# Sudaraka88/LDWeaver

Measured on AMD Instinct MI355X. Metric: MI SNP-pairs/sec, higher is better.
Workload: dtype i8

## Files before the change

### include/ldweaver_amd_debug.h

```cpp
#ifndef LDWEAVER_AMD_DEBUG_H
#define LDWEAVER_AMD_DEBUG_H

#include "ldweaver_amd.h"

#ifdef __cplusplus
extern "C" {
#endif

#define LDW_ENGINE_MFMA 0
#define LDW_ENGINE_HIST 1
#define LDW_ENGINE_HIST_STATES 2

int ldw_build_info(void);
int ldw_ctx_last_timing(ldw_ctx *ctx, double ms_out[4]);
int ldw_ctx_counters(ldw_ctx *ctx, int64_t out[4]);
int ldw_ctx_counters2(ldw_ctx *ctx, int64_t out[8]);
int ldw_gemm_stats(ldw_ctx *ctx, double out[6], int reset);
int ldw_apx_info(ldw_ctx *ctx, double out[6]);

int ldw_hamming_stats(ldw_ctx *ctx, double out[8]);
int ldw_joint_tables(ldw_ctx *ctx, const int32_t *pair_a, const int32_t *pair_b, int64_t npairs,
                     int64_t *counts_out, int64_t *fixed_out, int *frac_bits_out);

int ldw_set_engine(ldw_ctx *ctx, int engine);
int ldw_set_overlap(ldw_ctx *ctx, int on);
int ldw_set_fused(ldw_ctx *ctx, int on);
int ldw_set_mixed(ldw_ctx *ctx, int on);
int ldw_set_path(ldw_ctx *ctx, int mode);
int ldw_set_select(ldw_ctx *ctx, int mode);
int ldw_set_screen(ldw_ctx *ctx, int mode);
int ldw_set_prune(ldw_ctx *ctx, int on);
int ldw_set_pair_cap(uint32_t cap);
int ldw_reset_speculation(ldw_ctx *ctx);

int ldw_path_report(ldw_ctx *ctx, int64_t out[8], char *gate, int capacity);
int ldw_pair_form_report(ldw_ctx *ctx, int64_t out[5]);
int ldw_prune_report(ldw_ctx *ctx, int64_t out[4]);
int ldw_span_report(ldw_ctx *ctx, int64_t out[4]);
int ldw_overflow_report(ldw_ctx *ctx, int64_t out[4]);
int ldw_slot_report(ldw_ctx *ctx, int64_t out[6]);
int ldw_resource_report(int64_t out[5]);

int ldw_snp_bounds(ldw_ctx *ctx, double *out, int64_t capacity);
int ldw_debug_violations(ldw_ctx *ctx, double *out);
int ldw_debug_tab11(ldw_ctx *ctx, double W, double lo, double delta, double eta, double sprime, int32_t *out, double *cbin_out);
int ldw_debug_apx_params(ldw_ctx *ctx, double out[20], int64_t *vfixed_out, int64_t *vapx_out, int64_t capacity);
int ldw_debug_rows(ldw_ctx *ctx, int32_t *row0_out, uint32_t *slot_meta_out, int64_t capacity);
int ldw_debug_apx_gemm(ldw_ctx *ctx, const int32_t *rows_t, int nrt, const int32_t *rows_f, int nrf, int32_t *out);
int ldw_debug_apx_gemm_list(ldw_ctx *ctx, const int32_t *rows_t, int nrt, const int32_t *rows_f, int nrf, int grid_wgs, int32_t *out);
int ldw_debug_screen_bound(ldw_ctx *ctx, int kind, int na, int nb, int64_t n, const int64_t *g, const int64_t *pa, const int64_t *pb, const float *pX, const float *pY,
                           const double *rr, const uint32_t *masks, const double params[20], float *out, double *out64);

int ldw_debug_plot_panels(ldw_ctx *ctx, const double *x, const double *y, const double *srp, const uint8_t *layer, const uint8_t *panel, int64_t n,
                          int on_device, const ldw_plot_opts *opts, int n_panels, int32_t W, int32_t H, uint8_t *rgb_out, double *stats_out,
                          int64_t *scratch_bytes_out, double *ms_out);
int ldw_debug_plot_xy_panel(ldw_ctx *ctx, const double *x, const double *y, const uint8_t *cls, int64_t n, int on_device, const double *line_x,
                            const double *line_y, int64_t n_line, const ldw_plot_xy_opts *opts, int32_t W, int32_t H, uint8_t *rgb_out, double *stats_out,
                            double *ms_out);
int ldw_debug_plot_colours(int kind, const double *t, int64_t n, uint8_t *rgb_out);
int ldw_debug_plot_capsules(ldw_ctx *ctx, const ldw_capsule *caps, int64_t n_caps, int32_t W, int32_t H, uint8_t *rgb_out, double *ms_out);
int ldw_debug_plot_marks(ldw_ctx *ctx, const ldw_capsule *caps, int64_t n_caps, const ldw_rect *rects, int64_t n_rects, int32_t W, int32_t H, uint8_t *rgb_out,
                         double *ms_out);
int ldw_debug_plot_tree(ldw_ctx *ctx, int32_t W, int32_t H, const int32_t *panel, const ldw_bar *bars, int64_t n_bars, uint32_t bar_rgb, const uint8_t *levels,
                        int64_t n_tips, const uint32_t *palette, const int32_t *band_rect, int32_t n_bands, uint8_t *rgb_out, double *ms_out);
int ldw_links_grep_stats(ldw_ctx *ctx, double *out8);
int ldw_tsv_stats(ldw_ctx *ctx, double *out10);
int ldw_tsv_set_variant(ldw_ctx *ctx, int variant);

#ifdef __cplusplus
}
#endif
#endif
```

### ldweaver_amd/_lib.py

```python
from __future__ import annotations

import ctypes as C
import os

import numpy as np

_HERE = os.path.dirname(os.path.abspath(__file__))
LIB_PATH = os.environ.get("LDW_AMD_LIB") or os.path.join(_HERE, "libldweaver_amd.so")

LDW_OK = 0
LDW_ERR_ARG, LDW_ERR_HIP, LDW_ERR_STATE, LDW_ERR_NOGPU, LDW_ERR_SIZE = 1, 2, 3, 4, 5
QUIRK_REFERENCE, QUIRK_INTENDED = 0, 1
MI_SR_ROWS_STAY = 1
ENGINE_MFMA, ENGINE_HIST, ENGINE_HIST_STATES = 0, 1, 2
COL_INT32, COL_INT64, COL_DOUBLE, COL_STR = 0, 1, 2, 3


class LdwError(RuntimeError):
    def __init__(self, code: int, msg: str):
        super().__init__(f"libldweaver_amd error {code}: {msg}")
        self.code = code


PLOT_SR_CLUST, PLOT_SR_COMBI, PLOT_LR, PLOT_LDMAP = 0, 1, 2, 3
# ... 112 lines not shown
    "ldw_png_write": (C.c_int, [C.c_char_p, _p, C.c_int32, C.c_int32, C.c_int, C.POINTER(_i64)]),
    "ldw_plot_scatter": (C.c_int, [_p, _p, _p, _p, _p, _p, _i64, C.c_int, _p, C.c_int, _p, C.c_char_p, _p, C.POINTER(_i64)]),
    "ldw_plot_links": (C.c_int, [_p, C.c_int, C.c_int, _p, C.c_char_p, _p, C.POINTER(_i64)]),
    "ldw_plot_heatmap": (C.c_int, [_p, _p, C.c_int32, C.c_int, C.c_char_p, C.c_char_p, _p]),
    "ldw_plot_ldmap": (C.c_int, [_p, C.c_int32, C.c_int32, C.c_int32, C.c_char_p, C.c_char_p, _p, _p, _p, _p, _i64]),
    "ldw_plot_xy_layout_get": (C.c_int, [C.c_int, C.c_int, C.c_double, C.c_double, C.c_double, C.c_double, _p]),
    "ldw_plot_xy": (C.c_int, [_p, _p, _p, _p, _i64, C.c_int, _p, _p, _i64, _p, C.c_char_p, C.c_char_p, C.c_char_p, C.c_char_p, _p, C.POINTER(_i64)]),
    "ldw_plot_network": (C.c_int, [_p, _p, _i64, C.c_int32, C.c_int32, _p, _p, C.c_int32, C.c_char_p, _p, _p, C.c_int32, C.c_int32, C.c_char_p, _p, _p]),
    "ldw_plot_tanglegram": (C.c_int, [_p, _p, _i64, _p, _i64, C.c_int32, C.c_int32, _p, _p, C.c_int32, C.c_char_p, C.c_int32, C.c_char_p, _p, _p]),
    "ldw_plot_tree": (C.c_int, [_p, C.c_int32, C.c_int32, _p, _p, _i64, C.c_uint32, _p, _i64, _p, _p, C.c_int32, _p, C.c_char_p, _p, _p, _p, _p, _p, C.c_int32,
                                C.c_char_p, _p, _p]),
    "ldw_nj_tree": (C.c_int, [_p, _p, _i64, _p, _p]),
    "ldw_nj_bootstrap": (C.c_int, [_p, _p, _i64, _i64, _p, _p, _p, _p, _p]),
    "ldw_tree_parsimony": (C.c_int, [_p, _p, _p, _i64, C.c_int32, _p, _p]),
    "ldw_tree_states": (C.c_int, [_p, _p, _p, _i64, C.c_int32, _p, _i64, _p]),
    "ldw_tree_cochanges": (C.c_int, [_p, _p, _p, _i64, C.c_int32, _p, _p, _i64, _p, _p, _p]),
    "ldw_seq_clusters": (C.c_int, [_p, _p, C.c_int32, _p, _p]),
    "ldw_links_stratified": (C.c_int, [_p, _p, _p, _i64, _p, C.c_int32, _p, _p, _p, _p, _p, _p, C.POINTER(C.c_int)]),
    "ldw_links_permuted": (C.c_int, [_p, _p, _p, _i64, _p, C.c_int32, C.c_int32, C.c_uint64, _p, _p, _p, _p, _p, _p, C.POINTER(_i64), C.POINTER(C.c_int)]),
    "ldw_tsv_probe": (C.c_int, [C.c_char_p, C.c_int, C.POINTER(C.c_int32), C.POINTER(C.c_int32)]),
    "ldw_tsv_read": (C.c_int, [_p, C.c_char_p, C.c_int, C.c_int32, _i64, C.POINTER(_i64), C.POINTER(_i64), C.POINTER(C.c_uint32)]),
    "ldw_tsv_columns": (C.c_int, [_p, C.POINTER(_p), C.POINTER(_i64), C.POINTER(C.c_int32), C.POINTER(_i64)]),
    "ldw_tsv_fetch": (C.c_int, [_p, C.c_int32, _p, _i64, C.c_int]),
    "ldw_set_positions": (C.c_int, [_p, _p, _i64, C.c_double]),
    "ldw_links_load": (C.c_int, [_p, C.c_int, C.c_int32, C.c_int32, C.c_int32, C.c_int32, C.c_double, C.c_int32, C.POINTER(_i64)]),
    "ldw_links_grep": (C.c_int, [_p, C.c_char_p, _p, _p, C.c_int32, C.c_int32, _i64, C.POINTER(_i64), C.POINTER(_i64), C.POINTER(_i64)]),
    "ldw_links_grep_fetch": (C.c_int, [_p, _i64, _i64, _p, _p, _p, _p, _p]),
    "ldw_compare_to_row": (C.c_int, [_p, _i64, _i64, _p, _i64, _p]),
    "ldw_vec_pos_match": (C.c_int, [_p, _i64, _p, _i64, _p]),
    "ldw_compare_triplet": (C.c_int, [_p, _p, _i64, C.c_double, C.POINTER(C.c_int)]),
    "ldw_fast_intersect": (C.c_int, [_p, _i64, _p, _i64, _p, C.POINTER(_i64)]),
}
_SIGS_DEBUG = {
    "ldw_build_info": (C.c_int, []),
    "ldw_ctx_last_timing": (C.c_int, [_p, _p]),
    "ldw_ctx_counters": (C.c_int, [_p, _p]),
    "ldw_ctx_counters2": (C.c_int, [_p, _p]),
    "ldw_gemm_stats": (C.c_int, [_p, _p, C.c_int]),
    "ldw_apx_info": (C.c_int, [_p, _p]),
    "ldw_hamming_stats": (C.c_int, [_p, _p]),
    "ldw_joint_tables": (C.c_int, [_p, _p, _p, _i64, _p, _p, _p]),
    "ldw_set_engine": (C.c_int, [_p, C.c_int]),
    "ldw_set_overlap": (C.c_int, [_p, C.c_int]),
    "ldw_set_fused": (C.c_int, [_p, C.c_int]),
    "ldw_set_mixed": (C.c_int, [_p, C.c_int]),
    "ldw_set_path": (C.c_int, [_p, C.c_int]),
    "ldw_set_select": (C.c_int, [_p, C.c_int]),
    "ldw_set_screen": (C.c_int, [_p, C.c_int]),
    "ldw_set_prune": (C.c_int, [_p, C.c_int]),
    "ldw_set_pair_cap": (C.c_int, [C.c_uint32]),
    "ldw_reset_speculation": (C.c_int, [_p]),
    "ldw_path_report": (C.c_int, [_p, _p, C.c_char_p, C.c_int]),
    "ldw_pair_form_report": (C.c_int, [_p, _p]),
    "ldw_prune_report": (C.c_int, [_p, _p]),
    "ldw_span_report": (C.c_int, [_p, _p]),
    "ldw_overflow_report": (C.c_int, [_p, _p]),
    "ldw_slot_report": (C.c_int, [_p, _p]),
    "ldw_resource_report": (C.c_int, [_p]),
    "ldw_snp_bounds": (C.c_int, [_p, _p, C.c_int64]),
    "ldw_debug_violations": (C.c_int, [_p, _p]),
    "ldw_debug_tab11": (C.c_int, [_p, C.c_double, C.c_double, C.c_double, C.c_double, C.c_double, _p, _p]),
    "ldw_debug_apx_params": (C.c_int, [_p, _p, _p, _p, _i64]),
    "ldw_debug_rows": (C.c_int, [_p, _p, _p, _i64]),
    "ldw_debug_apx_gemm": (C.c_int, [_p, _p, C.c_int, _p, C.c_int, _p]),
    "ldw_debug_apx_gemm_list": (C.c_int, [_p, _p, C.c_int, _p, C.c_int, C.c_int, _p]),
    "ldw_debug_screen_bound": (C.c_int, [_p, C.c_int, C.c_int, C.c_int, _i64, _p, _p, _p, _p, _p, _p, _p, _p, _p, _p]),
    "ldw_debug_plot_panels": (C.c_int, [_p, _p, _p, _p, _p, _p, _i64, C.c_int, _p, C.c_int, C.c_int32, C.c_int32, _p, _p, C.POINTER(_i64), _p]),
    "ldw_debug_plot_xy_panel": (C.c_int, [_p, _p, _p, _p, _i64, C.c_int, _p, _p, _i64, _p, C.c_int32, C.c_int32, _p, _p, _p]),
    "ldw_debug_plot_colours": (C.c_int, [C.c_int, _p, _i64, _p]),
    "ldw_debug_plot_capsules": (C.c_int, [_p, _p, _i64, C.c_int32, C.c_int32, _p, _p]),
    "ldw_debug_plot_marks": (C.c_int, [_p, _p, _i64, _p, _i64, C.c_int32, C.c_int32, _p, _p]),
    "ldw_debug_plot_tree": (C.c_int, [_p, C.c_int32, C.c_int32, _p, _p, _i64, C.c_uint32, _p, _i64, _p, _p, C.c_int32, _p, _p]),
    "ldw_links_grep_stats": (C.c_int, [_p, _p]),
    "ldw_tsv_stats": (C.c_int, [_p, _p]),
    "ldw_tsv_set_variant": (C.c_int, [_p, C.c_int]),
}
_SIGS = {**_SIGS_API, **_SIGS_DEBUG}
_SIGS_BY_HEADER = {"ldweaver_amd.h": _SIGS_API, "ldweaver_amd_debug.h": _SIGS_DEBUG}


def declared_symbols(header: str | None = None):
    return sorted(_SIGS if header is None else _SIGS_BY_HEADER[header])


def lib():
    global _lib
    if _lib is None:
        if not os.path.exists(LIB_PATH):
            raise FileNotFoundError(
                f"{LIB_PATH} not found: build it with `make -C ldweaver_amd/csrc` or "
                "`python -c 'import __graft_entry__ as g; g.build()'` — there is no CPU fallback")
        try:
            import torch
        except ImportError:
            pass
        l = C.CDLL(LIB_PATH)
        for name, (res, args) in _SIGS.items():
            fn = getattr(l, name)
            fn.restype = res
            fn.argtypes = args
        _lib = l
    return _lib


def has_experiments() -> bool:
    return bool(lib().ldw_build_info() & 1)
# ... 23 lines not shown
```

### ldweaver_amd/csrc/ldw_api.hip

```cpp
#include <algorithm>
#include <atomic>
#include <chrono>
#include <cmath>
#include <cstdio>
#include <cstdlib>
#include <cstring>

#include <thread>
#include "ldw_internal.h"
#include "ldw_dev.h"
#include "ldw_fasta.h"
#include "ldw_links_read.h"
#include "ldw_slots.h"

namespace ldw {
int check_gpu(ldw_ctx *ctx) {
    LDW_REQUIRE(ctx != nullptr, LDW_ERR_ARG, "null context");
    LDW_HIP(hipSetDevice(ctx->device));
    return LDW_OK;
}
}

using namespace ldw;

// ... 316 lines not shown
        LDW_HIP(c->stream.ensure(hipStreamNonBlocking));
    }
    return LDW_OK;
}

int ldw_ctx_sync(ldw_ctx *c) {
    if (int rc = check_gpu(c)) return rc;
    LDW_HIP(hipStreamSynchronize(c->stream));
    return LDW_OK;
}

int ldw_ctx_last_timing(ldw_ctx *c, double ms_out[4]) {
    LDW_REQUIRE(c && ms_out, LDW_ERR_ARG, "ldw_ctx_last_timing: null argument");
    for (int i = 0; i < 4; ++i) ms_out[i] = c->last_ms[i];
    return LDW_OK;
}

static int ctx_counters(ldw_ctx *c, int64_t *out, int n, const char *who) {
    LDW_REQUIRE(c && out, LDW_ERR_ARG, "%s: null argument", who);
    const ldw::PassCounters &k = c->cnt;
    const int64_t all[8] = {k.spec_misses, 0 , k.blocks_run, k.screen_violations, k.mixed_blocks, k.apx_blocks, k.apx_units_listed, k.apx_pairs_listed};
    std::copy(all, all + n, out);
    return LDW_OK;
}
int ldw_ctx_counters2(ldw_ctx *c, int64_t out[8]) { return ctx_counters(c, out, 8, "ldw_ctx_counters2"); }
int ldw_ctx_counters(ldw_ctx *c, int64_t out[4]) { return ctx_counters(c, out, 4, "ldw_ctx_counters"); }

int ldw_reset_speculation(ldw_ctx *c) {
    LDW_REQUIRE(c, LDW_ERR_ARG, "null context");
    c->spec.reset();
    return LDW_OK;
}

int ldw_path_report(ldw_ctx *c, int64_t out[8], char *gate, int capacity) {
    LDW_REQUIRE(c && out, LDW_ERR_ARG, "ldw_path_report: null argument");
    out[0] = c->cnt.apx_blocks;
    out[1] = c->cnt.mixed_blocks;
    out[2] = c->cnt.blocks_run - c->cnt.apx_blocks - c->cnt.mixed_blocks + c->cnt.spec_misses + c->cnt.generic_blocks;
    out[3] = 0;
    out[4] = c->cnt.spec_misses;
    out[5] = c->cnt.probe_blocks;
    out[6] = c->cnt.apx_pairs_listed;
    out[7] = c->cnt.apx_units_listed;
    if (gate && capacity > 0) snprintf(gate, (size_t)capacity, "%s", c->apx.gate(c->wts.have_weights));
    return LDW_OK;
}

int ldw_pair_form_report(ldw_ctx *c, int64_t out[5]) {
    LDW_REQUIRE(c && out, LDW_ERR_ARG, "ldw_pair_form_report: null argument");
    for (int i = 0; i < 5; ++i) out[i] = c->cnt.form_launches[i];
    return LDW_OK;
}

int ldw_set_prune(ldw_ctx *c, int on) {
    LDW_REQUIRE(c, LDW_ERR_ARG, "null context");
    c->knobs.prune = on != 0;
    return LDW_OK;
}

int ldw_prune_report(ldw_ctx *c, int64_t out[4]) {
    LDW_REQUIRE(c && out, LDW_ERR_ARG, "ldw_prune_report: null argument");
    out[0] = c->cnt.sorted_blocks;
    out[1] = c->cnt.apx_waves_skipped;
    out[2] = c->cnt.apx_waves_total;
    out[3] = c->knobs.prune ? 1 : 0;
    return LDW_OK;
}

int ldw_snp_bounds(ldw_ctx *c, double *out, int64_t capacity) {
    if (int rc = check_gpu(c)) return rc;
    LDW_REQUIRE(out, LDW_ERR_ARG, "ldw_snp_bounds: null argument");
    if (int rc = ldw::ensure_rows(c)) return rc;
    LDW_REQUIRE(capacity >= 4 * c->L, LDW_ERR_ARG, "ldw_snp_bounds: capacity %lld < 4 L = %lld", (long long)capacity, (long long)(4 * c->L));
    LDW_HIP(hipMemcpyAsync(out, c->rows.snp_sup.p, (size_t)c->L * 32, hipMemcpyDeviceToHost, c->stream));
    LDW_HIP(hipStreamSynchronize(c->stream));
    return LDW_OK;
}

int ldw_set_select(ldw_ctx *c, int mode) {
    LDW_REQUIRE(c && (mode == 0 || mode == 1), LDW_ERR_ARG, "ldw_set_select: mode must be 0 (auto) or 1 (radix sorts)");
    c->knobs.select_mode = mode;
    return LDW_OK;
}

int ldw_set_path(ldw_ctx *c, int mode) {
    LDW_REQUIRE(c && mode >= 0 && mode <= 2, LDW_ERR_ARG, "ldw_set_path: mode must be 0 (auto), 1 (limb GEMM paths) or 2 (approximate GEMM path)");
    c->knobs.path_mode = mode;
    return LDW_OK;
}

int ldw_apx_info(ldw_ctx *c, double out[6]) {
    LDW_REQUIRE(c && out, LDW_ERR_ARG, "ldw_apx_info: null argument");
    out[0] = c->apx.apx_ok ? 1.0 : 0.0;
    out[1] = c->apx.apx_delta;
    out[2] = (double)c->apx.n_classes;
    out[3] = (double)c->apx.n_pop_segs;
    out[4] = (double)c->apx.apx_transitions;
    out[5] = (double)c->apx.apx_e_last;
    return LDW_OK;
}

int ldw_gemm_stats(ldw_ctx *c, double out[6], int reset) {
    LDW_REQUIRE(c && out, LDW_ERR_ARG, "ldw_gemm_stats: null argument");
    for (int k = 0; k < 6; ++k) {
        out[k] = c->cnt.gemm_stat[k];
        if (reset) c->cnt.gemm_stat[k] = 0;
// ... 552 lines not shown
```

### ldweaver_amd/csrc/ldw_apx.hip

```cpp
#include <algorithm>
#include <cmath>
#include <cstdlib>
#include <cstring>

#include "ldw_apx.h"
#include "ldw_dev.h"

using namespace ldw;

namespace ldw {

namespace {
constexpr int64_t APX_PROD_CAP = 12000;
struct ProdTable {
    std::vector<int32_t> val;
    std::vector<uint8_t> a, b;
    ProdTable() {
        std::vector<std::pair<int32_t, std::pair<uint8_t, uint8_t>>> all;
        for (int x = 0; x <= 127; ++x)
            for (int y = x; y <= 127; ++y) all.push_back({x * y, {(uint8_t)x, (uint8_t)y}});
        std::sort(all.begin(), all.end());
        for (auto &e : all)
            if (val.empty() || val.back() != e.first) {
                val.push_back(e.first);
// ... 645 lines not shown
#pragma unroll
            for (int j = 0; j < CB; ++j) t2[j] = (!GENB || j < nb) ? tr[j][w] : 0u;
            const int s0 = s_wbeg[w] & 0x7FFFFFFF, s1 = s_wbeg[w + 1] & 0x7FFFFFFF;
            for (int sg = s0; sg < s1; ++sg) {
                const PopSeg seg = s_segs[sg];
#pragma unroll
                for (int j = 0; j < CB; ++j)
#pragma unroll
                    for (int i = 0; i < CA; ++i)
                        if (!GENB || (i < na && j < nb)) s[j][i] += (int64_t)((uint64_t)__popc(f2[i] & t2[j] & seg.mask) * (uint64_t)seg.V);
            }
        }
#pragma unroll
        for (int j = 0; j < CB; ++j)
#pragma unroll
            for (int i = 0; i < CA; ++i) {
                int64_t v = s[j][i];
                if (!GENB || (i < na && j < nb)) {
#pragma unroll
                    for (int off = 32; off > 0; off >>= 1) v += __shfl_xor(v, off);
                }
                if (lane == 0) P.sums[((int64_t)sub * A.pl_cap + idx) * 16 + j * 4 + i] = v;
            }
    }
}

template <bool GEN>
__global__ __launch_bounds__(256) void k_pair_sums(PairArgs P) {
    extern __shared__ __attribute__((aligned(16))) uint8_t pop_smem[];
    int32_t *s_wbeg = reinterpret_cast<int32_t *>(pop_smem);
    PopSeg *s_segs = reinterpret_cast<PopSeg *>(pop_smem + (((size_t)P.nwords + 4) * 4 + 15) / 16 * 16);
    const int path = GEN ? 4 : (int)blockIdx.z;
    if (blockIdx.x * 4u >= P.A.pl_n[path * PAIR_SHARDS + (int)blockIdx.y]) return;
    if (P.seg_in_lds) {
        for (int i = threadIdx.x; i < P.nwords + 1; i += 256) s_wbeg[i] = P.wbeg[i];
        for (int i = threadIdx.x; i < P.nseg; i += 256) s_segs[i] = P.segs[i];
        __syncthreads();
    } else {
        s_wbeg = const_cast<int32_t *>(P.wbeg);
        s_segs = const_cast<PopSeg *>(P.segs);
    }
    if constexpr (GEN) {
        pair_sums_body<4, 4>(P, 4, s_wbeg, s_segs);
    } else {
        switch (path) {
            case 0: pair_sums_body<1, 1>(P, 0, s_wbeg, s_segs); break;
            case 1: pair_sums_body<2, 1>(P, 1, s_wbeg, s_segs); break;
            case 2: pair_sums_body<1, 2>(P, 2, s_wbeg, s_segs); break;
            default: pair_sums_body<2, 2>(P, 3, s_wbeg, s_segs); break;
        }
    }
}

template <int CA, int CB>
__device__ __forceinline__ void pair_sums_bits_body(const PairArgs &P, int path, const int64_t *sVT, int stride) {
    constexpr bool GENB = CA == 4 && CB == 4;
    const EpiArgs &A = P.A;
    const int sub = path * PAIR_SHARDS + (int)blockIdx.y;
    unsigned int n = A.pl_n[sub];
    n = n > A.pl_cap ? A.pl_cap : n;
    const int lane = threadIdx.x & 63;
    const PairEnt *list = A.pl_pairs + (int64_t)sub * A.pl_cap;
    for (unsigned int idx = blockIdx.x * 4u + (threadIdx.x >> 6); idx < n; idx += gridDim.x * 4u) {
        const PairEnt e = list[idx];
        const uint32_t era = (uint32_t)__builtin_amdgcn_readfirstlane((int)e.ra), erb = (uint32_t)__builtin_amdgcn_readfirstlane((int)e.rb);
        const int r0a = (int)(era & 0x1FFFFFFFu), na = (int)(era >> 29), r0b = (int)(erb & 0x1FFFFFFFu), nb = (int)(erb >> 29);
        const uint32_t *fr[CA], *tr[CB];
#pragma unroll
        for (int i = 0; i < CA; ++i) fr[i] = reinterpret_cast<const uint32_t *>(P.Mbits + (int64_t)(i < na ? r0a + i : P.zero_row) * P.KW);
#pragma unroll
        for (int j = 0; j < CB; ++j) tr[j] = reinterpret_cast<const uint32_t *>(P.Mbits + (int64_t)(j < nb ? r0b + j : P.zero_row) * P.KW);
        int64_t s[CB][CA];
#pragma unroll
        for (int j = 0; j < CB; ++j)
#pragma unroll
            for (int i = 0; i < CA; ++i) s[j][i] = 0;
        for (int w = lane; w < P.nwords; w += 64) {
            uint32_t f[CA], t[CB], uf = 0u, ut = 0u;
#pragma unroll
            for (int i = 0; i < CA; ++i) {
                f[i] = (!GENB || i < na) ? fr[i][w] : 0u;
                uf |= f[i];
            }
#pragma unroll
            for (int j = 0; j < CB; ++j) {
                t[j] = (!GENB || j < nb) ? tr[j][w] : 0u;
                ut |= t[j];
            }
            uint32_t u = uf & ut;
            while (u) {
                const int b = __builtin_ctz(u);
                u &= u - 1u;
                const int64_t v = sVT[b * stride + w];
#pragma unroll
                for (int j = 0; j < CB; ++j)
#pragma unroll
                    for (int i = 0; i < CA; ++i)
                        if (CA * CB == 1 || (((f[i] & t[j]) >> b) & 1u)) s[j][i] += v;
            }
        }
#pragma unroll
        for (int j = 0; j < CB; ++j)
#pragma unroll
            for (int i = 0; i < CA; ++i) {
                int64_t v = s[j][i];
                if (!GENB || (i < na && j < nb)) {
// ... 115 lines not shown
    __shared__ unsigned int s_hist[LDW_SPAN_MAX * PAIR_HWIN];
    for (int i = threadIdx.x; i < LDW_SPAN_MAX * PAIR_HWIN; i += 256) s_hist[i] = 0u;
    __syncthreads();
    switch (blockIdx.z) {
        case 0: pair_mi_body<1, 1>(P, 0, s_hist); break;
        case 1: pair_mi_body<2, 1>(P, 1, s_hist); break;
        case 2: pair_mi_body<1, 2>(P, 2, s_hist); break;
        case 3: pair_mi_body<2, 2>(P, 3, s_hist); break;
        default: pair_mi_body<0, 0>(P, 4, s_hist); break;
    }
    __syncthreads();
    const int hb0 = P.A.E.spec_B > 0 ? P.A.E.spec_B : 0;
    if (P.A.span) {
        for (int i = threadIdx.x; i < P.A.span * PAIR_HWIN; i += 256) {
            const int k = i / PAIR_HWIN, w = i - k * PAIR_HWIN;
            if (s_hist[i] != 0u && hb0 + w < NBINS) atomicAdd(&P.A.sseg[k].ghist[hb0 + w], (unsigned long long)s_hist[i]);
        }
        return;
    }
    if (threadIdx.x < PAIR_HWIN && s_hist[threadIdx.x] != 0u && hb0 + (int)threadIdx.x < NBINS)
        atomicAdd(&P.ghist[hb0 + threadIdx.x], (unsigned long long)s_hist[threadIdx.x]);
}

int launch_pairs_exact(ldw_ctx *c, const EpiArgs &A, unsigned long long *ghist, int64_t *sums, hipStream_t st) {
    PairArgs P;
    memset(&P, 0, sizeof(P));
    P.Mbits = c->rows.Mbits.as<uint64_t>();
    P.KW = c->KW;
    P.nwords = (int)(c->KW * 2);
    P.nseg = c->apx.n_pop_segs;
    P.segs = c->apx.pop_segs.as<PopSeg>();
    P.wbeg = c->apx.pop_wbeg.as<int32_t>();
    P.row0 = c->rows.row0.as<int32_t>();
    P.zero_row = (int32_t)c->rows.R;
    P.sums = sums;
    P.A = A;
    P.ghist = ghist;
    size_t lds = (((size_t)P.nwords + 4) * 4 + 15) / 16 * 16 + (size_t)P.nseg * sizeof(PopSeg);
    P.seg_in_lds = lds <= 60000 ? 1 : 0;
    if (!P.seg_in_lds) lds = 0;
    const int stride = (P.nwords + 31) / 32 * 32;
    const size_t lds_bits = (size_t)32 * stride * 8;
    const bool bits_off = getenv("LDW_NO_PAIR_BITS") != nullptr;
    const bool many_classes = !P.seg_in_lds || P.nseg >= 8 * P.nwords;
    if (many_classes && !bits_off && lds_bits <= 160 * 1024 && c->apx.pop_vpos.p) {
        if (lds_bits > 64 * 1024 && !c->pair_bits_attr) {
            LDW_HIP(hipFuncSetAttribute(reinterpret_cast<const void *>(k_pair_sums_bits<false>), hipFuncAttributeMaxDynamicSharedMemorySize, 160 * 1024));
            LDW_HIP(hipFuncSetAttribute(reinterpret_cast<const void *>(k_pair_sums_bits<true>), hipFuncAttributeMaxDynamicSharedMemorySize, 160 * 1024));
            c->pair_bits_attr = true;
        }
        hipLaunchKernelGGL(k_pair_sums_bits<false>, dim3(256, PAIR_SHARDS, 4), dim3(256), lds_bits, st, P, c->apx.pop_vpos.as<int64_t>(), stride);
        hipLaunchKernelGGL(k_pair_sums_bits<true>, dim3(256, PAIR_SHARDS, 1), dim3(256), lds_bits, st, P, c->apx.pop_vpos.as<int64_t>(), stride);
        c->cnt.form_launches[lds_bits > 64 * 1024 ? 1 : 0] += 2;
    } else {
        static const unsigned gx_env = [] { const char *e = getenv("LDW_PAIR_GRID"); return e ? (unsigned)atoi(e) : 0u; }();
        hipLaunchKernelGGL(k_pair_sums<false>, dim3(gx_env ? gx_env : 512u, PAIR_SHARDS, 4), dim3(256), lds, st, P);
        hipLaunchKernelGGL(k_pair_sums<true>, dim3(gx_env ? gx_env : 1024u, PAIR_SHARDS, 1), dim3(256), lds, st, P);
        c->cnt.form_launches[P.seg_in_lds ? 2 : 3] += 2;
    }
    hipLaunchKernelGGL(k_pair_mi, dim3(64, PAIR_SHARDS, PAIR_PATHS), dim3(256), 0, st, P);
    LDW_HIP(hipGetLastError());
    return LDW_OK;
}

}

namespace ldw {
void warm_apx() {
    hipFuncAttributes a;
    (void)hipFuncGetAttributes(&a, reinterpret_cast<const void *>(&k_pack_panel));
    (void)hipGetLastError();
}
}
```

### ldweaver_amd/csrc/ldw_internal.h

```cpp
#pragma once
#include <hip/hip_runtime.h>
#include <stdint.h>
#include <stdlib.h>
#include <algorithm>
#include <string>
#include <atomic>
#include <chrono>
#include <memory>
#include <mutex>
#include <thread>
#include <vector>

#include "../../include/ldweaver_amd.h"
#include "../../include/ldweaver_amd_debug.h"
#include "ldw_own.h"

#define LDW_NSLOT 3


namespace ldw {

void set_error(const char *fmt, ...);
int hip_fail(hipError_t e, const char *what, const char *file, int line);

// ... 143 lines not shown
    bool hi_ready = false;
    DevBuf slot_papx;
    DevBuf counts;
    DevBuf pfix_state;
    DevBuf snp_sup;
    std::vector<int32_t> h_row0;
    std::vector<uint32_t> h_slot_meta;
    std::vector<int32_t> h_counts;
    std::vector<int64_t> h_minor_w;
    std::vector<int32_t> h_span_bad;
    std::mutex order_mtx;
    std::vector<std::unique_ptr<OrderCache>> order_cache;
    void invalidate() { rows_ready = false; }
    void rebuilt() { rows_ready = true, hi_ready = false, order_cache.clear(); }
};

struct Speculation {
    bool spec_seen[2] = {false, false};
    bool spec_probed[2] = {false, false};
    int spec_hist[2][6] = {{0, 0, 0, 0, 0, 0}, {0, 0, 0, 0, 0, 0}};
    int spec_hist_n[2] = {0, 0};
    bool spec_small[2] = {false, false};
    int spec_B_next[2] = {-1, -1};
    bool maybe_off = false;
    DevBuf tab11[2];
    double tab11_lo[2] = {0, 0};
    int tab11_cur[2] = {0, 0};
    float tab11_c = 0;
    int tab11_nb = 0;
    void forget_guesses() {
        spec_B_next[0] = spec_B_next[1] = -1;
        spec_seen[0] = spec_seen[1] = spec_probed[0] = spec_probed[1] = false;
        spec_hist_n[0] = spec_hist_n[1] = 0;
    }
    void drop_tables() { tab11_lo[0] = tab11_lo[1] = 0; }
    void reset() { forget_guesses(), drop_tables(), maybe_off = false; }
};

struct LinkTables {
    DevBuf sr_a, sr_b, sr_mi, lr_a, lr_b, lr_mi;
    int64_t n_sr = 0, n_lr = 0;
    int64_t blk_capacity = 0, blk_cursor = 0;
    std::vector<BlockStat> stats;
    std::vector<int32_t> multi_owner;
    void drop_deal() { multi_owner.clear(); }
    void new_pass() { n_sr = n_lr = 0, stats.clear(), drop_deal(); }
    void replaced(KeptLinks &kept) { kept.invalidate(), stats.clear(), drop_deal(); }
    void clear(KeptLinks &kept) { n_sr = n_lr = 0, replaced(kept); }
};

struct PassCounters {
    int64_t apx_blocks = 0, apx_units_listed = 0, apx_pairs_listed = 0, probe_blocks = 0, generic_blocks = 0;
    int64_t form_launches[5] = {0, 0, 0, 0, 0};
    int64_t apx_waves_skipped = 0, apx_waves_total = 0;
    int64_t tab11_builds = 0;
    int64_t slot_grown = 0;
    int64_t maybe_entries = 0;
    int64_t pair_list_overflows = 0, maybe_overflows = 0;
    int64_t span_items = 0, span_blocks = 0, span_fallbacks = 0;
    std::atomic<int64_t> sorted_blocks{0};
    int64_t spec_misses = 0, blocks_run = 0, screen_violations = 0, mixed_blocks = 0;
    double gemm_stat[6] = {0, 0, 0, 0, 0, 0};
};

struct Knobs {
    int engine = LDW_ENGINE_MFMA;
    int path_mode = 0;
    int select_mode = 0;
    int mixed = 1;
    bool prune = true;
    bool span_on = true;
    int span_max = 8;
    bool overlap = true;
    int screen = 1;
};

inline bool host_timing() {
    static const bool on = getenv("LDW_HOST_TIMING") != nullptr;
    return on;
}
struct HostClock {
    using Point = std::chrono::steady_clock::time_point;
    static Point now() { return std::chrono::steady_clock::now(); }
    static double ms(Point a, Point b) { return std::chrono::duration<double, std::milli>(b - a).count(); }
    static double us(Point a, Point b) { return std::chrono::duration<double, std::micro>(b - a).count(); }
};
}

struct ldw_ctx {
    int device = 0;
    int n_cu = 0;
    ldw::Stream stream;
    ldw::Stream copy_stream, gemm_stream;
    ldw::Stream lr_st;
    bool streams_ready = false;
    ldw::Event ev[6];
    double last_ms[4] = {0, 0, 0, 0};

    int64_t L = 0, N = 0, Npad = 0;
    int64_t KW = 0;
    ldw::DevBuf states;
    ldw::DevBuf chars;
    int64_t cN = 0, cL = 0;
    void *fasta = nullptr;
    void *out = nullptr;
    void *tsv = nullptr;
// ... 126 lines not shown
```

### ldweaver_amd/engine.py

```python
from __future__ import annotations

import ctypes as C
import errno
import os

import numpy as np

from . import _lib as L

ANNOT_REC = 12


def fasta_check(code: int, path):
    if code == L.LDW_OK:
        return
    msg = L.lib().ldw_last_error().decode("utf-8", "replace")
    if "does not contain any sequences" in msg:
        raise ValueError("File does not contain any sequences!")
    if "sequences are of different lengths" in msg:
        raise ValueError("Error! sequences are of different lengths!")
    if "cannot open" in msg:
        raise FileNotFoundError(errno.ENOENT, msg, str(path)) if not os.path.exists(path) else OSError(msg)
    raise L.LdwError(code, msg)

# ... 24 lines not shown
            self.close()
        except Exception:
            pass

    def __enter__(self):
        return self

    def __exit__(self, *a):
        self.close()

    def set_stream(self, stream):
        L.check(L.lib().ldw_ctx_set_stream(self._ctx, C.c_void_p(int(stream) if stream else 0)))

    def sync(self):
        L.check(L.lib().ldw_ctx_sync(self._ctx))

    def last_timing(self):
        t = np.zeros(4)
        L.check(L.lib().ldw_ctx_last_timing(self._ctx, L.ptr(t)))
        return dict(gemm_ms=t[0], epilogue_ms=t[1], select_ms=t[2], total_ms=t[3])

    def gemm_stats(self, reset: bool = False):
        v = np.zeros(6)
        L.check(L.lib().ldw_gemm_stats(self._ctx, L.ptr(v), int(reset)))
        return dict(apx_launches=int(v[0]), apx_ops=float(v[1]), bits_launches=int(v[2]), bits_ops=float(v[3]), band_launches=int(v[4]),
                    apx_table_launches=int(v[5]))

    def hamming_stats(self):
        v = np.zeros(8)
        L.check(L.lib().ldw_hamming_stats(self._ctx, L.ptr(v)))
        return dict(columns=int(v[0]), k_padded=int(v[1]), pre_ms=float(v[2]), gemm_ms=float(v[3]), post_ms=float(v[4]), pre_bytes=float(v[5]), post_bytes=float(v[6]),
                    wall_ms=float(v[7]))

    def counters(self):
        v = np.zeros(8, dtype=np.int64)
        L.check(L.lib().ldw_ctx_counters2(self._ctx, L.ptr(v)))
        return dict(spec_misses=int(v[0]), fused_blocks=int(v[1]), unfused_blocks=int(v[2]), screen_violations=int(v[3]),
                    mixed_blocks=int(v[4]), apx_blocks=int(v[5]), apx_units_listed=int(v[6]), apx_pairs_listed=int(v[7]))

    def reset_speculation(self):
        L.check(L.lib().ldw_reset_speculation(self._ctx))

    def path_report(self):
        v = np.zeros(8, dtype=np.int64)
        buf = C.create_string_buffer(200)
        L.check(L.lib().ldw_path_report(self._ctx, L.ptr(v), buf, 200))
        return dict(apx_blocks=int(v[0]), mixed_blocks=int(v[1]), plain_blocks=int(v[2]), fused_blocks=int(v[3]), spec_misses=int(v[4]),
                    probe_blocks=int(v[5]), pairs_listed=int(v[6]), units_listed=int(v[7]), apx_gate=buf.value.decode())

    def form_report(self):
        v = np.zeros(5, dtype=np.int64)
        L.check(L.lib().ldw_pair_form_report(self._ctx, L.ptr(v)))
        return dict(bits_lds64=int(v[0]), bits_lds160=int(v[1]), classwise_lds=int(v[2]), classwise_global=int(v[3]), fill_rows_global=int(v[4]))

    def set_prune(self, on: bool):
        L.check(L.lib().ldw_set_prune(self._ctx, int(bool(on))))

    def prune_report(self):
        v = np.zeros(4, dtype=np.int64)
        L.check(L.lib().ldw_prune_report(self._ctx, L.ptr(v)))
        return dict(ordered_blocks=int(v[0]), tiles_pruned=int(v[1]), tiles_total=int(v[2]), on=bool(v[3]))

    def sr_pairs(self, blocks, sr_dist: float, n_rows: int | None = None):
        import torch
        bl = L.as_c(blocks, np.int32).reshape(-1, 4)
        n = C.c_int64(0)
        if n_rows is None:
            L.check(L.lib().ldw_sr_pairs_fill(self._ctx, L.ptr(bl), len(bl), float(sr_dist), None, None, 0, C.byref(n)))
            n_rows = int(n.value)
        dev = torch.device("cuda", self.device)
        a = torch.empty(max(1, n_rows), dtype=torch.int32, device=dev)
        b = torch.empty(max(1, n_rows), dtype=torch.int32, device=dev)
        torch.cuda.synchronize(dev)
        L.check(L.lib().ldw_sr_pairs_fill(self._ctx, L.ptr(bl), len(bl), float(sr_dist), C.c_void_p(a.data_ptr()), C.c_void_p(b.data_ptr()), n_rows, C.byref(n)))
        assert int(n.value) == n_rows, (int(n.value), n_rows)
        return a[:n_rows], b[:n_rows]

    def set_span(self, on: bool, max_blocks: int = 0, corners: bool = False, diag_split: bool = False):
        L.check(L.lib().ldw_set_span(self._ctx, (1 if on else 0) | (2 if (on and corners) else 0) | (4 if (on and diag_split) else 0), int(max_blocks)))

    def span_report(self):
        v = np.zeros(4, dtype=np.int64)
        L.check(L.lib().ldw_span_report(self._ctx, L.ptr(v)))
        return dict(spans=int(v[0]), blocks=int(v[1]), redone=int(v[2]), on=bool(v[3]))

    def overflow_report(self):
        v = np.zeros(4, dtype=np.int64)
        L.check(L.lib().ldw_overflow_report(self._ctx, L.ptr(v)))
        return dict(pair_list=int(v[0]), maybe_list=int(v[1]), maybe_off=bool(v[2]), maybe_entries=int(v[3]))

    def slot_report(self):
        v = np.zeros(6, dtype=np.int64)
        L.check(L.lib().ldw_slot_report(self._ctx, L.ptr(v)))
        return dict(grown=int(v[0]), units=int(v[1]), packs=int(v[2]), pairs=int(v[3]), bins=int(v[4]), mini=int(v[5]))

    @staticmethod
    def set_pair_cap(cap: int):
        L.check(L.lib().ldw_set_pair_cap(int(cap)))

    def snp_bounds(self):
        out = np.zeros(4 * self.L)
        L.check(L.lib().ldw_snp_bounds(self._ctx, L.ptr(out), out.size))
        return out.reshape(self.L, 2, 2)

    APX_PARAM_NAMES = ("F", "e_last", "delta", "lost_units", "total_fixed", "neff", "apx_EG", "apx_dfac", "apx_s1", "apx_c1", "apx_W", "apx_unit", "scr_scale",
                       "scr_shift_exact", "scr_scale_exact", "flags", "lo_abs_sum", "lo_bound", "apx_MU", "nlimbs")
# ... 938 lines not shown
```

Measured before the change: 172.9 billion.

## Add quarter-wave pair-sum kernel with persistent grid and row prefetch

Adds a new pair-sums kernel in which each 16-lane quarter of a wavefront handles one pair, reducing across lanes with DPP row operations instead of using a whole wave per pair. It runs a persistent grid sized per compute unit, caches a few segment masks per word in registers, and software-prefetches the next pair's rows. It becomes the default when segments fit in LDS, with the old wave-per-pair kernel kept behind an environment switch. The aim is better lane utilisation for short rows and hidden load latency, at the cost of higher register pressure and lower occupancy.

```diff
diff --git a/include/ldweaver_amd_debug.h b/include/ldweaver_amd_debug.h
--- a/include/ldweaver_amd_debug.h
+++ b/include/ldweaver_amd_debug.h
@@ -35,6 +35,7 @@
 
 int ldw_path_report(ldw_ctx *ctx, int64_t out[8], char *gate, int capacity);
 int ldw_pair_form_report(ldw_ctx *ctx, int64_t out[5]);
+int ldw_pair_kernel_report(ldw_ctx *ctx, int64_t out[2]);
 int ldw_prune_report(ldw_ctx *ctx, int64_t out[4]);
 int ldw_span_report(ldw_ctx *ctx, int64_t out[4]);
 int ldw_overflow_report(ldw_ctx *ctx, int64_t out[4]);
diff --git a/ldweaver_amd/_lib.py b/ldweaver_amd/_lib.py
--- a/ldweaver_amd/_lib.py
+++ b/ldweaver_amd/_lib.py
@@ -188,6 +188,7 @@
     "ldw_reset_speculation": (C.c_int, [_p]),
     "ldw_path_report": (C.c_int, [_p, _p, C.c_char_p, C.c_int]),
     "ldw_pair_form_report": (C.c_int, [_p, _p]),
+    "ldw_pair_kernel_report": (C.c_int, [_p, _p]),
     "ldw_prune_report": (C.c_int, [_p, _p]),
     "ldw_span_report": (C.c_int, [_p, _p]),
     "ldw_overflow_report": (C.c_int, [_p, _p]),
diff --git a/ldweaver_amd/csrc/ldw_api.hip b/ldweaver_amd/csrc/ldw_api.hip
--- a/ldweaver_amd/csrc/ldw_api.hip
+++ b/ldweaver_amd/csrc/ldw_api.hip
@@ -392,6 +392,12 @@
     return LDW_OK;
 }
 
+int ldw_pair_kernel_report(ldw_ctx *c, int64_t out[2]) {
+    LDW_REQUIRE(c && out, LDW_ERR_ARG, "ldw_pair_kernel_report: null argument");
+    for (int i = 0; i < 2; ++i) out[i] = c->cnt.pair_kernel_launches[i];
+    return LDW_OK;
+}
+
 int ldw_set_prune(ldw_ctx *c, int on) {
     LDW_REQUIRE(c, LDW_ERR_ARG, "null context");
     c->knobs.prune = on != 0;
diff --git a/ldweaver_amd/csrc/ldw_apx.hip b/ldweaver_amd/csrc/ldw_apx.hip
--- a/ldweaver_amd/csrc/ldw_apx.hip
+++ b/ldweaver_amd/csrc/ldw_apx.hip
@@ -721,6 +721,245 @@
     }
 }
 
+constexpr int PQ_KQ = 5, PQ_KS = 2;
+constexpr int PQ_WGS_PER_CU = 2;
+
+template <int CTRL>
+__device__ __forceinline__ int64_t dpp_add64(int64_t v) {
+    const uint32_t lo = (uint32_t)__builtin_amdgcn_update_dpp(0, (int)(uint32_t)v, CTRL, 0xF, 0xF, false);
+    const uint32_t hi = (uint32_t)__builtin_amdgcn_update_dpp(0, (int)(uint32_t)((uint64_t)v >> 32), CTRL, 0xF, 0xF, false);
+    return v + (int64_t)(((uint64_t)hi << 32) | (uint64_t)lo);
+}
+__device__ __forceinline__ int64_t row16_sum(int64_t v) {
+    v = dpp_add64<0xB1>(v);
+    v = dpp_add64<0x4E>(v);
+    v = dpp_add64<0x141>(v);
+    v = dpp_add64<0x140>(v);
+    return v;
+}
+
+template <int CA, int CB, bool PREF>
+__device__ __forceinline__ void pair_sums_q_body(const PairArgs &P, int path, const int32_t *s_wbeg, const PopSeg *s_segs) {
+    constexpr bool GENB = CA == 4 && CB == 4;
+    constexpr int KQ = PQ_KQ, KS = PQ_KS;
+    const EpiArgs &A = P.A;
+    const int lane = threadIdx.x & 63, l = lane & 15, grp = lane >> 4;
+    unsigned int pre[PAIR_SHARDS + 1];
+    pre[0] = 0u;
+#pragma unroll
+    for (int s = 0; s < PAIR_SHARDS; ++s) {
+        const unsigned int n = A.pl_n[path * PAIR_SHARDS + s];
+        pre[s + 1] = pre[s] + (n > A.pl_cap ? A.pl_cap : n);
+    }
+    const unsigned int total = pre[PAIR_SHARDS];
+    const unsigned int nwv = gridDim.x * 4u;
+    unsigned int t = blockIdx.x * 4u + (threadIdx.x >> 6);
+    if (4u * t >= total) return;
+    const PairEnt *lists = A.pl_pairs + (int64_t)path * PAIR_SHARDS * A.pl_cap;
+    auto locate = [&](unsigned int p, int &shard, unsigned int &idx) {
+        shard = 0;
+        unsigned int base = 0u;
+#pragma unroll
+        for (int s = 1; s < PAIR_SHARDS; ++s)
+            if (p >= pre[s]) shard = s, base = pre[s];
+        idx = p - base;
+    };
+    auto load_ent = [&](unsigned int tt) -> uint2 {
+        const unsigned int p = 4u * tt + (unsigned int)grp;
+        if (p >= total) return make_uint2(0u, 0u);
+        int shard;
+        unsigned int idx;
+        locate(p, shard, idx);
+        const PairEnt *e = lists + (int64_t)shard * A.pl_cap + idx;
+        return make_uint2(e->ra, e->rb);
+    };
+    auto row_ptr = [&](uint32_t r, int i) -> const uint2 * {
+        const int r0 = (int)(r & 0x1FFFFFFFu), n = (int)(r >> 29);
+        return reinterpret_cast<const uint2 *>(P.Mbits + (int64_t)(i < n ? r0 + i : P.zero_row) * P.KW);
+    };
+    auto issue_rows = [&](uint2 e, uint2 (&f)[KQ][CA], uint2 (&tt)[KQ][CB]) {
+        const int na = (int)(e.x >> 29), nb = (int)(e.y >> 29);
+#pragma unroll
+        for (int i = 0; i < CA; ++i) {
+            const uint2 *fr = row_ptr(e.x, i);
+#pragma unroll
+            for (int k = 0; k < KQ; ++k) f[k][i] = (32 * k + 2 * l < P.nwords && (!GENB || i < na)) ? fr[16 * k + l] : make_uint2(0u, 0u);
+        }
+#pragma unroll
+        for (int j = 0; j < CB; ++j) {
+            const uint2 *tr = row_ptr(e.y, j);
+#pragma unroll
+            for (int k = 0; k < KQ; ++k) tt[k][j] = (32 * k + 2 * l < P.nwords && (!GENB || j < nb)) ? tr[16 * k + l] : make_uint2(0u, 0u);
+        }
+    };
+    uint32_t smask[KQ][2][KS];
+    int64_t sV[KQ][2][KS];
+    uint32_t more = 0u;
+#pragma unroll
+    for (int k = 0; k < KQ; ++k)
+#pragma unroll
+        for (int h = 0; h < 2; ++h) {
+            const int w = 32 * k + 2 * l + h;
+            int s0 = 0, s1 = 0;
+            if (w < P.nwords) {
+                s0 = s_wbeg[w] & 0x7FFFFFFF;
+                s1 = s_wbeg[w + 1] & 0x7FFFFFFF;
+            }
+            const bool mr = s1 - s0 > KS;
+            if (mr) more |= 1u << (2 * k + h);
+#pragma unroll
+            for (int q = 0; q < KS; ++q) {
+                const bool on = s0 + q < s1 && !mr;
+                smask[k][h][q] = on ? s_segs[s0 + q].mask : 0u;
+                sV[k][h][q] = on ? s_segs[s0 + q].V : 0;
+            }
+        }
+    uint2 e_cur = load_ent(t);
+    uint2 f[KQ][CA], tt[KQ][CB];
+    issue_rows(e_cur, f, tt);
+    unsigned int tn = t + nwv;
+    uint2 e_nx = load_ent(tn);
+    for (;;) {
+        const bool has_nx = 4u * tn < total;
+        uint2 fn[KQ][CA], tnx[KQ][CB];
+        uint2 e_nx2 = make_uint2(0u, 0u);
+        if (PREF && has_nx) {
+            issue_rows(e_nx, fn, tnx);
+            e_nx2 = load_ent(tn + nwv);
+        }
+        const int na = (int)(e_cur.x >> 29), nb = (int)(e_cur.y >> 29);
+        int namax = CA, nbmax = CB;
+        if constexpr (GENB) {
+            namax = 1 + (__ballot(na >= 2) != 0ull) + (__ballot(na >= 3) != 0ull) + (__ballot(na >= 4) != 0ull);
+            nbmax = 1 + (__ballot(nb >= 2) != 0ull) + (__ballot(nb >= 3) != 0ull) + (__ballot(nb >= 4) != 0ull);
+        }
+        int64_t s[CB][CA];
+#pragma unroll
+        for (int j = 0; j < CB; ++j)
+#pragma unroll
+            for (int i = 0; i < CA; ++i) s[j][i] = 0;
+#pragma unroll
+        for (int k = 0; k < KQ; ++k) {
+            if (32 * k >= P.nwords) break;
+#pragma unroll
+            for (int h = 0; h < 2; ++h) {
+                uint32_t fw[CA], tw[CB];
+#pragma unroll
+                for (int i = 0; i < CA; ++i) fw[i] = h ? f[k][i].y : f[k][i].x;
+#pragma unroll
+                for (int j = 0; j < CB; ++j) tw[j] = h ? tt[k][j].y : tt[k][j].x;
+#pragma unroll
+                for (int q = 0; q < KS; ++q)
+#pragma unroll
+                    for (int j = 0; j < CB; ++j)
+#pragma unroll
+                        for (int i = 0; i < CA; ++i)
+                            if (!GENB || (i < namax && j < nbmax)) s[j][i] += (int64_t)((uint64_t)__popc(fw[i] & tw[j] & smask[k][h][q]) * (uint64_t)sV[k][h][q]);
+                if ((more >> (2 * k + h)) & 1u) {
+                    const int w = 32 * k + 2 * l + h;
+                    const int s0 = s_wbeg[w] & 0x7FFFFFFF, s1 = s_wbeg[w + 1] & 0x7FFFFFFF;
+                    for (int sg = s0; sg < s1; ++sg) {
+                        const PopSeg seg = s_segs[sg];
+#pragma unroll
+                        for (int j = 0; j < CB; ++j)
+#pragma unroll
+                            for (int i = 0; i < CA; ++i)
+                                if (!GENB || (i < namax && j < nbmax)) s[j][i] += (int64_t)((uint64_t)__popc(fw[i] & tw[j] & seg.mask) * (uint64_t)seg.V);
+                    }
+                }
+            }
+        }
+        if (32 * KQ < P.nwords) {
+            const uint2 *fr[CA], *tr[CB];
+#pragma unroll
+            for (int i = 0; i < CA; ++i) fr[i] = row_ptr(e_cur.x, i);
+#pragma unroll
+            for (int j = 0; j < CB; ++j) tr[j] = row_ptr(e_cur.y, j);
+            for (int w2 = 16 * KQ + l; 2 * w2 < P.nwords; w2 += 16) {
+                uint2 f2[CA], t2[CB];
+#pragma unroll
+                for (int i = 0; i < CA; ++i) f2[i] = fr[i][w2];
+#pragma unroll
+                for (int j = 0; j < CB; ++j) t2[j] = tr[j][w2];
+#pragma unroll
+                for (int h = 0; h < 2; ++h) {
+                    const int w = 2 * w2 + h;
+                    const int s0 = s_wbeg[w] & 0x7FFFFFFF, s1 = s_wbeg[w + 1] & 0x7FFFFFFF;
+                    for (int sg = s0; sg < s1; ++sg) {
+                        const PopSeg seg = s_segs[sg];
+#pragma unroll
+                        for (int j = 0; j < CB; ++j)
+#pragma unroll
+                            for (int i = 0; i < CA; ++i)
+                                if (!GENB || (i < namax && j < nbmax))
+                                    s[j][i] += (int64_t)((uint64_t)__popc((h ? f2[i].y : f2[i].x) & (h ? t2[j].y : t2[j].x) & seg.mask) * (uint64_t)seg.V);
+                    }
+                }
+            }
+        }
+#pragma unroll
+        for (int j = 0; j < CB; ++j)
+#pragma unroll
+            for (int i = 0; i < CA; ++i)
+                if (!GENB || (i < namax && j < nbmax)) s[j][i] = row16_sum(s[j][i]);
+        const unsigned int p = 4u * t + (unsigned int)grp;
+        if (l == 0 && p < total) {
+            int shard;
+            unsigned int idx;
+            locate(p, shard, idx);
+            int64_t *o = P.sums + ((int64_t)(path * PAIR_SHARDS + shard) * A.pl_cap + idx) * 16;
+#pragma unroll
+            for (int j = 0; j < CB; ++j)
+#pragma unroll
+                for (int i = 0; i < CA; ++i) o[j * 4 + i] = s[j][i];
+        }
+        if (!has_nx) break;
+        t = tn;
+        tn += nwv;
+        e_cur = e_nx;
+        if constexpr (PREF) {
+#pragma unroll
+            for (int k = 0; k < KQ; ++k) {
+#pragma unroll
+                for (int i = 0; i < CA; ++i) f[k][i] = fn[k][i];
+#pragma unroll
+                for (int j = 0; j < CB; ++j) tt[k][j] = tnx[k][j];
+            }
+            e_nx = e_nx2;
+        } else {
+            issue_rows(e_cur, f, tt);
+            e_nx = load_ent(tn);
+        }
+    }
+}
+
+template <bool GEN>
+__global__ __launch_bounds__(256) void k_pair_sums_q(PairArgs P) {
+    extern __shared__ __attribute__((aligned(16))) uint8_t pop_smem[];
+    int32_t *s_wbeg = reinterpret_cast<int32_t *>(pop_smem);
+    PopSeg *s_segs = reinterpret_cast<PopSeg *>(pop_smem + (((size_t)P.nwords + 4) * 4 + 15) / 16 * 16);
+    const int path = GEN ? 4 : (int)blockIdx.z;
+    unsigned int total = 0u;
+    for (int s = 0; s < PAIR_SHARDS; ++s) {
+        const unsigned int n = P.A.pl_n[path * PAIR_SHARDS + s];
+        total += n > P.A.pl_cap ? P.A.pl_cap : n;
+    }
+    if (blockIdx.x * 16u >= total) return;
+    for (int i = threadIdx.x; i < P.nwords + 1; i += 256) s_wbeg[i] = P.wbeg[i];
+    for (int i = threadIdx.x; i < P.nseg; i += 256) s_segs[i] = P.segs[i];
+    __syncthreads();
+    if constexpr (GEN) {
+        pair_sums_q_body<4, 4, false>(P, 4, s_wbeg, s_segs);
+    } else {
+        switch (path) {
+            case 0: pair_sums_q_body<1, 1, true>(P, 0, s_wbeg, s_segs); break;
+            case 1: pair_sums_q_body<2, 1, true>(P, 1, s_wbeg, s_segs); break;
+            case 2: pair_sums_q_body<1, 2, true>(P, 2, s_wbeg, s_segs); break;
+            default: pair_sums_q_body<2, 2, true>(P, 3, s_wbeg, s_segs); break;
+        }
+    }
+}
+
 template <int CA, int CB>
 __device__ __forceinline__ void pair_sums_bits_body(const PairArgs &P, int path, const int64_t *sVT, int stride) {
     constexpr bool GENB = CA == 4 && CB == 4;
@@ -942,7 +1181,15 @@
         hipLaunchKernelGGL(k_pair_sums_bits<false>, dim3(256, PAIR_SHARDS, 4), dim3(256), lds_bits, st, P, c->apx.pop_vpos.as<int64_t>(), stride);
         hipLaunchKernelGGL(k_pair_sums_bits<true>, dim3(256, PAIR_SHARDS, 1), dim3(256), lds_bits, st, P, c->apx.pop_vpos.as<int64_t>(), stride);
         c->cnt.form_launches[lds_bits > 64 * 1024 ? 1 : 0] += 2;
+    } else if (const char *wv = getenv("LDW_PAIR_WAVE"); P.seg_in_lds && !(wv && atoi(wv) != 0)) {
+        static const unsigned per_cu_env = [] { const char *e = getenv("LDW_PAIR_GRID"); return e ? (unsigned)atoi(e) : 0u; }();
+        const unsigned gx = (per_cu_env ? per_cu_env : (unsigned)PQ_WGS_PER_CU) * (unsigned)std::max(c->n_cu, 1);
+        hipLaunchKernelGGL(k_pair_sums_q<false>, dim3(gx, 1, 4), dim3(256), lds, st, P);
+        hipLaunchKernelGGL(k_pair_sums_q<true>, dim3(gx, 1, 1), dim3(256), lds, st, P);
+        c->cnt.form_launches[2] += 2;
+        c->cnt.pair_kernel_launches[0] += 2;
     } else {
+        c->cnt.pair_kernel_launches[1] += 2;
         static const unsigned gx_env = [] { const char *e = getenv("LDW_PAIR_GRID"); return e ? (unsigned)atoi(e) : 0u; }();
         hipLaunchKernelGGL(k_pair_sums<false>, dim3(gx_env ? gx_env : 512u, PAIR_SHARDS, 4), dim3(256), lds, st, P);
         hipLaunchKernelGGL(k_pair_sums<true>, dim3(gx_env ? gx_env : 1024u, PAIR_SHARDS, 1), dim3(256), lds, st, P);
diff --git a/ldweaver_amd/csrc/ldw_internal.h b/ldweaver_amd/csrc/ldw_internal.h
--- a/ldweaver_amd/csrc/ldw_internal.h
+++ b/ldweaver_amd/csrc/ldw_internal.h
@@ -219,6 +219,7 @@
 struct PassCounters {
     int64_t apx_blocks = 0, apx_units_listed = 0, apx_pairs_listed = 0, probe_blocks = 0, generic_blocks = 0;
     int64_t form_launches[5] = {0, 0, 0, 0, 0};
+    int64_t pair_kernel_launches[2] = {0, 0};
     int64_t apx_waves_skipped = 0, apx_waves_total = 0;
     int64_t tab11_builds = 0;
     int64_t slot_grown = 0;
diff --git a/ldweaver_amd/engine.py b/ldweaver_amd/engine.py
--- a/ldweaver_amd/engine.py
+++ b/ldweaver_amd/engine.py
@@ -100,6 +100,11 @@
         v = np.zeros(5, dtype=np.int64)
         L.check(L.lib().ldw_pair_form_report(self._ctx, L.ptr(v)))
         return dict(bits_lds64=int(v[0]), bits_lds160=int(v[1]), classwise_lds=int(v[2]), classwise_global=int(v[3]), fill_rows_global=int(v[4]))
+
+    def pair_kernel_report(self):
+        v = np.zeros(2, dtype=np.int64)
+        L.check(L.lib().ldw_pair_kernel_report(self._ctx, L.ptr(v)))
+        return dict(quarter_wave=int(v[0]), wave=int(v[1]))
 
     def set_prune(self, on: bool):
         L.check(L.lib().ldw_set_prune(self._ctx, int(bool(on))))
```

Result: faster. 177.4 billion, median of 6 (+2.6%).
